# TMElyralab/MuseV

Measured on NVIDIA H100. Metric: denoised frames/sec at 512x512, 16-frame window, 20 DDIM steps, higher is better.
Workload: dtype f16 (fp32 accumulate)

## Files before the change

musev_b200/csrc/conv_gemm.cu:

```cuda
#include "conv_gemm.cuh"

#include <dlfcn.h>
#include <stdio.h>
#include <stdlib.h>
#include <string.h>

#include <mutex>

#include "ptx.cuh"
#include "stats.cuh"

namespace mvb {

static constexpr int kMaxStages = 8;
static constexpr int kBlockM = 128;
static constexpr int kBlockK = 64;
static constexpr int kABytes = kBlockM * kBlockK * 2;
static constexpr int kAccLd = 132;
static constexpr int kAccBytes = 2 * 64 * kAccLd * 4;
static constexpr int kBiasBytes = 2 * 256 * 4;
static constexpr int kRingBytes = 227 * 1024 - kAccBytes - kBiasBytes - 1024  - 256 ;
static constexpr int kSmemBytes = kRingBytes + kAccBytes + kBiasBytes + 1024 + 256;
__device__ __forceinline__ float gelu_erf(float x) { return 0.5f * x * (1.f + erff(x * 0.70710678118654752440f)); }
__device__ __forceinline__ float silu(float x) { return __fdividef(x, 1.f + __expf(-x)); }
__device__ __forceinline__ float gelu_fast(float x) {
  const float z = fabsf(x) * 0.70710678118654752440f;
  const float t = __frcp_rn(fmaf(0.3275911f, z, 1.f));
  float poly = fmaf(1.061405429f, t, -1.453152027f);
  poly = fmaf(poly, t, 1.421413741f);
  poly = fmaf(poly, t, -0.284496736f);
  poly = fmaf(poly, t, 0.254829592f);
  poly *= t;
  float e;
  asm("ex2.approx.ftz.f32 %0, %1;" : "=f"(e) : "f"(-z * z * 1.4426950408889634f));
  const float erf_abs = fmaf(-poly, e, 1.f);
  const float erf_v = copysignf(erf_abs, x);
  return 0.5f * x * (1.f + erf_v);
}

__device__ __forceinline__ float rcp_approx(float x) {
  float y;
  asm("rcp.approx.ftz.f32 %0, %1;" : "=f"(y) : "f"(x));
  return y;
}
__device__ __forceinline__ F2 geglu2(F2 val, F2 gate) {
  float g0, g1;
  f2_get(gate, g0, g1);
  const F2 u = f2_make(fabsf(g0), fabsf(g1));
  float d0, d1;
  f2_get(f2_fma(u, f2_make(0.231641888f, 0.231641888f), f2_make(1.f, 1.f)), d0, d1);
  const F2 t = f2_make(rcp_approx(d0), rcp_approx(d1));
  F2 poly = f2_fma(t, f2_make(-0.5307027145f, -0.5307027145f), f2_make(0.7265760135f, 0.7265760135f));
  poly = f2_fma(poly, t, f2_make(-0.7107068705f, -0.7107068705f));
  poly = f2_fma(poly, t, f2_make(0.142248368f, 0.142248368f));
  poly = f2_fma(poly, t, f2_make(-0.127414796f, -0.127414796f));
  poly = f2_mul(poly, t);
  float a0, a1;
  f2_get(f2_mul(f2_mul(u, f2_make(-0.72134752044f, -0.72134752044f)), u), a0, a1);
  float e0, e1;
  asm("ex2.approx.ftz.f32 %0, %1;" : "=f"(e0) : "f"(a0));
  asm("ex2.approx.ftz.f32 %0, %1;" : "=f"(e1) : "f"(a1));
  const F2 gelu = f2_fma(u, f2_mul(poly, f2_make(e0, e1)), f2_make(fmaxf(g0, 0.f), fmaxf(g1, 0.f)));
  return f2_mul(val, gelu);
}

enum : int {
  kEpiGeneric = 0,
  kEpiPlain = 1,
  kEpiResidual = 2,
  kEpiGeglu = 3,
  kEpiAct = 4
};
__device__ __forceinline__ float gelu_act(float x, int act) {
  return act == 2 ? gelu_erf(x) : act == 3 ? __fdividef(x, 1.f + __expf(-1.702f * x)) : x;
}

struct AMaps {
  CUtensorMap m[4];
};

template <int kEpi, int BN>
__global__ void __launch_bounds__(384, 1)
conv_gemm_kernel(const __grid_constant__ AMaps tmA, const __grid_constant__ CUtensorMap tmB,
                 const __grid_constant__ ConvGemmParams p) {
  extern __shared__ uint8_t smem_raw[];
  uint8_t* smem = reinterpret_cast<uint8_t*>((reinterpret_cast<uintptr_t>(smem_raw) + 1023) & ~uintptr_t(1023));
  float* sacc = reinterpret_cast<float*>(smem + kRingBytes);
  float* sbias = reinterpret_cast<float*>(smem + kRingBytes + kAccBytes);
  uint64_t* bars = reinterpret_cast<uint64_t*>(smem + kRingBytes + kAccBytes + kBiasBytes);
  uint64_t* full = bars;
  uint64_t* empty = bars + kMaxStages;
  const int nstages = p.nstages;
  const int stage_bytes = p.stage_bytes;

  const int warp = threadIdx.x >> 5;
  const int lane = threadIdx.x & 31;

  if (threadIdx.x == 0) {
    tma_prefetch_desc(&tmA.m[0]);
    tma_prefetch_desc(&tmA.m[1]);
    tma_prefetch_desc(&tmA.m[2]);
    tma_prefetch_desc(&tmA.m[3]);
    tma_prefetch_desc(&tmB);
    for (int s = 0; s < kMaxStages; ++s) {
      mbar_init(&full[s], 1);
      mbar_init(&empty[s], 8);
    }
    fence_barrier_init();
  }
  __syncthreads();

  const int kb_per_tap = p.kb0 + p.kb1;
  const int num_kb = p.ntaps * kb_per_tap;
  const int tiles_m = p.tiles_w * p.tiles_h * p.tiles_n;
  const int num_units = tiles_m * p.tiles_nn;
  const uint32_t stage_tx = kABytes + (uint32_t)BN * kBlockK * 2;

  if (warp < 4) {
    setmaxnreg_dec<40>();
    if (warp == 0) {
      int stage = 0;
      uint32_t phase = 0;
      for (int unit = blockIdx.x; unit < num_units; unit += gridDim.x) {
        const int nt = unit % p.tiles_nn;
        const int mt = unit / p.tiles_nn;
        const int tw = mt % p.tiles_w;
        const int th = (mt / p.tiles_w) % p.tiles_h;
        const int tn = mt / (p.tiles_w * p.tiles_h);
        const int w0 = tw * p.bw, h0 = th * p.bh, n0 = tn * p.bn;
        int kcol = 0;
        const int ncoord = nt * BN;
        for (int tap = 0; tap < p.ntaps; ++tap) {
          const int xw = w0 + p.dx[tap], yh = h0 + p.dy[tap];
          const int src0 = p.tap_src[tap];
          for (int cb = 0; cb < kb_per_tap; ++cb, kcol += kBlockK) {
            const bool first = cb < p.kb0;
            const int src = src0 + (first ? 0 : 1);
            const int c0 = (first ? cb : cb - p.kb0) * kBlockK;
            const CUtensorMap* tm = &tmA.m[src];
            mbar_wait(&empty[stage], phase ^ 1);
            if (elect_one()) {
              uint8_t* sa = smem + stage * stage_bytes;
              uint8_t* sb = sa + kABytes;
              mbar_expect_tx(&full[stage], stage_tx);
              tma_load_4d(sa, tm, &full[stage], c0, xw, yh, n0);
              tma_load_2d(sb, &tmB, &full[stage], kcol, ncoord);
            }
            __syncwarp();
            if (++stage == nstages) { stage = 0; phase ^= 1; }
          }
        }
      }
    }
    return;
  }

  setmaxnreg_inc<232>();
  const int wg = (warp - 4) >> 2;
  const int t = threadIdx.x - 128 * (1 + wg);
  const int wq = t >> 5;
  const int row_local = t & 63;
  const int half = t >> 6;
  const int r = 64 * wg + row_local;
  float* acc_slice = sacc + wg * 64 * kAccLd;
  float* wbias = sbias + wg * 256;
  const bool use_res = (p.res != nullptr) && !p.geglu && !p.out_f32;
  const int acc_step = p.geglu ? 64 : 32;
  const uint64_t desc0_a = make_desc_k_sw128(smem_u32(smem) + (uint32_t)wg * 64 * 128);
  const uint64_t desc0_b = make_desc_k_sw128(smem_u32(smem) + kABytes);
  const uint32_t stage_step = (uint32_t)stage_bytes >> 4;
  int stage = 0;
  uint32_t phase = 0;
  float acc[BN / 2];

  for (int unit = blockIdx.x; unit < num_units; unit += gridDim.x) {
    const int nt = unit % p.tiles_nn;
    const int mt = unit / p.tiles_nn;
    const int tw = mt % p.tiles_w;
    const int th = (mt / p.tiles_w) % p.tiles_h;
    const int tn = mt / (p.tiles_w * p.tiles_h);
    const int ncol0 = nt * BN;

    int prev_stage = 0;
    for (int kb = 0; kb < num_kb; ++kb) {
      mbar_wait(&full[stage], phase);
      const uint64_t da = desc0_a + (uint64_t)((uint32_t)stage * stage_step);
      const uint64_t db = desc0_b + (uint64_t)((uint32_t)stage * stage_step);
      wgmma_fence();
      fence_regs(acc);
#pragma unroll
      for (int k = 0; k < kBlockK / 16; ++k)
        Wgmma<BN>::ss(acc, da + (uint64_t)(k * 2), db + (uint64_t)(k * 2), (kb | k) != 0);
      wgmma_commit();
      fence_regs(acc);
      if (kb > 0) {
        wgmma_wait<1>();
        fence_regs(acc);
        __syncwarp();
        if (lane == 0) mbar_arrive(&empty[prev_stage]);
      }
      prev_stage = stage;
      if (++stage == nstages) { stage = 0; phase ^= 1; }
    }
    wgmma_wait<0>();
    fence_regs(acc);
    __syncwarp();
    if (lane == 0) mbar_arrive(&empty[prev_stage]);

    const int rw = r % p.bw;
    const int rh = (r / p.bw) % p.bh;
    const int rn = r / (p.bw * p.bh);
    const int w = tw * p.bw + rw, h = th * p.bh + rh, n = tn * p.bn + rn;
    const bool row_ok = (w < p.W) && (h < p.H) && (n < p.NF);
    const long long m = ((long long)n * p.H + h) * p.W + w;
    const float* radd = (p.rowadd && row_ok) ? p.rowadd + (long long)(m / p.rows_per_group) * p.ld_rowadd : nullptr;
    const __half* res_row = use_res ? p.res + m * p.ld_res : nullptr;
    __half* out_row = reinterpret_cast<__half*>(p.out) + m * p.ldc;

    uint4 rcur[4] = {};
    auto load_res = [&](int c0, uint4 (&dst)[4]) {
      if (!use_res || !row_ok) return;
#pragma unroll
      for (int g = 0; g < 4; ++g) {
        const int nn = ncol0 + c0 + g * 8;
        if (c0 + g * 8 < BN && nn < p.N) dst[g] = __ldg(reinterpret_cast<const uint4*>(res_row + nn));
      }
    };
    named_bar_sync(1 + wg, 128);
    if constexpr (kEpi != kEpiGeneric && kEpi != kEpiAct) {
      for (int c = t; c < BN; c += 128) wbias[c] = (p.bias && ncol0 + c < p.N) ? __ldg(p.bias + ncol0 + c) : 0.f;
    }
#pragma unroll
    for (int u = 0; u < (BN + 127) / 128; ++u) {
      if (u > 0) named_bar_sync(1 + wg, 128);
#pragma unroll
      for (int i = 16 * u; i < 16 * u + 16 && i < BN / 8; ++i) {
        const int rr = 16 * wq + (lane >> 2);
        const int cc = 8 * (i - 16 * u) + 2 * (lane & 3);
        *reinterpret_cast<float2*>(acc_slice + rr * kAccLd + cc) = make_float2(acc[4 * i], acc[4 * i + 1]);
        *reinterpret_cast<float2*>(acc_slice + (rr + 8) * kAccLd + cc) = make_float2(acc[4 * i + 2], acc[4 * i + 3]);
      }
      named_bar_sync(1 + wg, 128);
      const int cend = (128 * u + 128 < BN) ? 128 * u + 128 : BN;
      for (int c0 = 128 * u + half * acc_step; c0 < cend; c0 += 2 * acc_step) {
        const float* srow = acc_slice + row_local * kAccLd + (c0 - 128 * u);
        auto ld32 = [&](const float* src, uint32_t (&v)[32]) {
#pragma unroll
          for (int k = 0; k < 8; ++k) {
            const float4 x = *reinterpret_cast<const float4*>(src + 4 * k);
            v[4 * k] = __float_as_uint(x.x); v[4 * k + 1] = __float_as_uint(x.y);
            v[4 * k + 2] = __float_as_uint(x.z); v[4 * k + 3] = __float_as_uint(x.w);
          }
        };
        load_res(c0, rcur);
        if constexpr (kEpi != kEpiGeneric && kEpi != kEpiAct) {
          const int nbase = ncol0 + c0;
          uint32_t v[32], vg[32];
          ld32(srow, v);
          if constexpr (kEpi == kEpiGeglu) ld32(srow + 32, vg);
          if (nbase < p.N && row_ok) {
            const F2 alpha2 = f2_make(p.alpha, p.alpha);
            const float* cbias = wbias + c0;
            const int oc = (kEpi == kEpiGeglu) ? nbase / 2 : nbase;
#pragma unroll
            for (int g = 0; g < 4; ++g) {
              uint32_t o[4];
              if constexpr (kEpi == kEpiGeglu) {
                const uint32_t* vv = (g < 2) ? v : vg;
                const int j0 = (g & 1) * 8;
#pragma unroll
                for (int e = 0; e < 4; ++e) {
                  const int j = j0 + 2 * e;
                  const float2 bv = *reinterpret_cast<const float2*>(cbias + (g >> 1) * 32 + j);
                  const float2 bg = *reinterpret_cast<const float2*>(cbias + (g >> 1) * 32 + 16 + j);
                  const F2 val = f2_add(f2_make(__uint_as_float(vv[j]), __uint_as_float(vv[j + 1])), f2_make(bv.x, bv.y));
                  const F2 gat = f2_add(f2_make(__uint_as_float(vv[16 + j]), __uint_as_float(vv[16 + j + 1])),
                                        f2_make(bg.x, bg.y));
                  float x0, x1;
                  f2_get(geglu2(val, gat), x0, x1);
                  const __half2 h2 = __floats2half2_rn(x0, x1);
                  o[e] = *reinterpret_cast<const uint32_t*>(&h2);
                }
              } else {
                float4 b0 = *reinterpret_cast<const float4*>(cbias + 8 * g);
                float4 b1 = *reinterpret_cast<const float4*>(cbias + 8 * g + 4);
                if (radd) {
                  const float4 a0 = __ldg(reinterpret_cast<const float4*>(radd + nbase) + 2 * g);
                  const float4 a1 = __ldg(reinterpret_cast<const float4*>(radd + nbase) + 2 * g + 1);
                  b0.x += a0.x; b0.y += a0.y; b0.z += a0.z; b0.w += a0.w;
                  b1.x += a1.x; b1.y += a1.y; b1.z += a1.z; b1.w += a1.w;
                }
                const float bb[8] = {b0.x, b0.y, b0.z, b0.w, b1.x, b1.y, b1.z, b1.w};
                const __half2* rh2 = reinterpret_cast<const __half2*>(&rcur[g]);
#pragma unroll
                for (int e = 0; e < 4; ++e) {
                  const int j = g * 8 + 2 * e;
                  F2 x = f2_add(f2_make(__uint_as_float(v[j]), __uint_as_float(v[j + 1])), f2_make(bb[2 * e], bb[2 * e + 1]));
                  if constexpr (kEpi == kEpiResidual) {
                    const float2 rr = __half22float2(rh2[e]);
                    x = f2_fma(x, alpha2, f2_make(rr.x, rr.y));
                  }
                  float x0, x1;
                  f2_get(x, x0, x1);
                  const __half2 h2 = __floats2half2_rn(x0, x1);
                  o[e] = *reinterpret_cast<const uint32_t*>(&h2);
                }
              }
              *reinterpret_cast<uint4*>(out_row + oc + 8 * g) = make_uint4(o[0], o[1], o[2], o[3]);
            }
          }
        } else {
          float f[32];
          const int nbase = ncol0 + c0;
          if (p.geglu) {
            uint32_t va[32], vb[32];
            ld32(srow, va);
            ld32(srow + 32, vb);
#pragma unroll
            for (int hsel = 0; hsel < 2; ++hsel) {
              const uint32_t* v = hsel ? vb : va;
              const int nb = nbase + hsel * 32;
#pragma unroll
              for (int j4 = 0; j4 < 4; ++j4) {
                const bool bok = p.bias && nb < p.N;
                const float4 bv = bok ? __ldg(reinterpret_cast<const float4*>(p.bias + nb) + j4) : make_float4(0, 0, 0, 0);
                const float4 bg = bok ? __ldg(reinterpret_cast<const float4*>(p.bias + nb + 16) + j4) : make_float4(0, 0, 0, 0);
                const int j = j4 * 4;
                const F2 v01 = f2_add(f2_make(__uint_as_float(v[j]), __uint_as_float(v[j + 1])), f2_make(bv.x, bv.y));
                const F2 v23 = f2_add(f2_make(__uint_as_float(v[j + 2]), __uint_as_float(v[j + 3])), f2_make(bv.z, bv.w));
                const F2 g01 = f2_add(f2_make(__uint_as_float(v[16 + j]), __uint_as_float(v[16 + j + 1])), f2_make(bg.x, bg.y));
                const F2 g23 = f2_add(f2_make(__uint_as_float(v[16 + j + 2]), __uint_as_float(v[16 + j + 3])), f2_make(bg.z, bg.w));
                f2_get(geglu2(v01, g01), f[hsel * 16 + j], f[hsel * 16 + j + 1]);
                f2_get(geglu2(v23, g23), f[hsel * 16 + j + 2], f[hsel * 16 + j + 3]);
              }
            }
          } else {
            uint32_t v[32];
            ld32(srow, v);
            if (nbase + 32 <= p.N) {
#pragma unroll
              for (int g = 0; g < 8; ++g) {
                float4 b = p.bias ? __ldg(reinterpret_cast<const float4*>(p.bias + nbase) + g) : make_float4(0, 0, 0, 0);
                if (radd) {
                  const float4 a4 = __ldg(reinterpret_cast<const float4*>(radd + nbase) + g);
                  b.x += a4.x; b.y += a4.y; b.z += a4.z; b.w += a4.w;
                }
                f[g * 4 + 0] = __uint_as_float(v[g * 4 + 0]) + b.x;
                f[g * 4 + 1] = __uint_as_float(v[g * 4 + 1]) + b.y;
                f[g * 4 + 2] = __uint_as_float(v[g * 4 + 2]) + b.z;
                f[g * 4 + 3] = __uint_as_float(v[g * 4 + 3]) + b.w;
              }
            } else {
#pragma unroll
              for (int j = 0; j < 32; ++j) {
                const int nn = nbase + j;
                float x = __uint_as_float(v[j]);
                if (nn < p.N) {
                  if (p.bias) x += __ldg(p.bias + nn);
                  if (radd) x += __ldg(radd + nn);
                }
                f[j] = x;
              }
            }
          }
          if (row_ok) {
            if (p.out_f32) {
#pragma unroll
              for (int g = 0; g < 8; ++g) {
                const int nn = nbase + g * 4;
                if (nn < p.N) {
                  float4 o4;
                  o4.x = f[g * 4 + 0] * p.alpha; o4.y = f[g * 4 + 1] * p.alpha;
                  o4.z = f[g * 4 + 2] * p.alpha; o4.w = f[g * 4 + 3] * p.alpha;
                  if (p.act == 1) { o4.x = silu(o4.x); o4.y = silu(o4.y); o4.z = silu(o4.z); o4.w = silu(o4.w); }
                  if constexpr (kEpi == kEpiAct) {
                    o4.x = gelu_act(o4.x, p.act); o4.y = gelu_act(o4.y, p.act);
                    o4.z = gelu_act(o4.z, p.act); o4.w = gelu_act(o4.w, p.act);
                  }
                  *reinterpret_cast<float4*>(reinterpret_cast<float*>(p.out) + m * p.ldc + nn) = o4;
                }
              }
            } else {
              const int oc = p.geglu ? nbase / 2 : nbase;
              const int ncols = p.geglu ? p.N / 2 : p.N;
#pragma unroll
              for (int g = 0; g < 4; ++g) {
                if (oc + 8 * g >= ncols) continue;
                __align__(16) __half o[8];
                const __half* rh8 = reinterpret_cast<const __half*>(&rcur[g]);
#pragma unroll
                for (int j = 0; j < 8; ++j) {
                  float x = f[g * 8 + j];
                  if (!p.geglu) {
                    x *= p.alpha;
                    if (use_res) x = fmaf(p.beta, __half2float(rh8[j]), x);
                    if (p.act == 1) x = silu(x);
                    if constexpr (kEpi == kEpiAct) x = gelu_act(x, p.act);
                  }
                  o[j] = __float2half_rn(x);
                }
                *reinterpret_cast<uint4*>(out_row + oc + 8 * g) = *reinterpret_cast<const uint4*>(o);
              }
            }
          }
        }
      }
    }
  }
}

typedef CUresult (*EncodeTiledFn)(CUtensorMap*, CUtensorMapDataType, cuuint32_t, void*, const cuuint64_t*,
                                  const cuuint64_t*, const cuuint32_t*, const cuuint32_t*, CUtensorMapInterleave,
                                  CUtensorMapSwizzle, CUtensorMapL2promotion, CUtensorMapFloatOOBfill);

EncodeTiledFn get_encode_fn() {
  static EncodeTiledFn fn = nullptr;
  static bool tried = false;
  if (!tried) {
    tried = true;
    void* h = dlopen("libcuda.so.1", RTLD_NOW | RTLD_GLOBAL);
    if (!h) h = dlopen("libcuda.so", RTLD_NOW | RTLD_GLOBAL);
    if (h) fn = reinterpret_cast<EncodeTiledFn>(dlsym(h, "cuTensorMapEncodeTiled"));
  }
  return fn;
}

namespace {
struct MapKey {
  uint64_t ptr, d[4], s[3];
  uint32_t box[4], rank, swz;
  bool operator==(const MapKey& o) const { return memcmp(this, &o, sizeof(MapKey)) == 0; }
};
struct MapSlot {
  MapKey key;
  CUtensorMap map;
  bool used;
};
static_assert(sizeof(MapKey) == 88, "MapKey is compared and hashed bytewise: no padding allowed");
static_assert(sizeof(MapSlot) % 64 == 0, "slots keep the 64-byte alignment of CUtensorMap");
constexpr uint32_t kMapSlots = 1u << 14;
std::mutex g_map_mutex;
MapSlot* g_map_slots = nullptr;
uint32_t g_map_count = 0;
unsigned long long g_map_hits = 0, g_map_misses = 0;

uint64_t hash_key(const MapKey& k) {
  const uint64_t* w = reinterpret_cast<const uint64_t*>(&k);
  uint64_t h = 0x9e3779b97f4a7c15ull;
  for (size_t i = 0; i < sizeof(MapKey) / 8; ++i) {
    h ^= w[i] + 0x9e3779b97f4a7c15ull + (h << 6) + (h >> 2);
    h *= 0xff51afd7ed558ccdull;
    h ^= h >> 33;
  }
  return h;
}
bool cache_enabled() {
  static const bool on = !(getenv("MVB_TMAP_CACHE") && atoi(getenv("MVB_TMAP_CACHE")) == 0);
  return on;
}
// ... 92 lines not shown
      }
    }
  }
}

static const int kBlockNs[4] = {64, 128, 160, 256};

static int pick_block_n(int N, int geglu, int gelu, long long tiles_m, int num_sms) {
  int best = 0;
  double best_cost = 1e30;
  for (int i = 3; i >= 0; --i) {
    const int bn = kBlockNs[i];
    if (geglu && (bn % 64)) continue;
    if (gelu && bn == 256) continue;
    const int tn = ceil_div(N, bn);
    const long long tiles = tiles_m * tn;
    const long long waves = (tiles + num_sms - 1) / num_sms;
    const double cost = (double)waves * (bn + 24.0);
    if (cost < best_cost - 1e-9) { best_cost = cost; best = bn; }
  }
  return best;
}

static cudaError_t launch_common(cudaStream_t stream, const CUtensorMap* maps, int nmaps, ConvGemmParams& p,
                                 const __half* wt, long long ktot, const Epilogue& ep, int num_sms, const char** err) {
  typedef void (*KernelFn)(const AMaps, const CUtensorMap, const ConvGemmParams);
#define MVB_GEMM_ROW(BN) \
  {conv_gemm_kernel<kEpiGeneric, BN>, conv_gemm_kernel<kEpiPlain, BN>, conv_gemm_kernel<kEpiResidual, BN>, \
   conv_gemm_kernel<kEpiGeglu, BN>, conv_gemm_kernel<kEpiAct, BN>}
  static const KernelFn kernels[4][5] = {MVB_GEMM_ROW(64), MVB_GEMM_ROW(128), MVB_GEMM_ROW(160),
                                         {conv_gemm_kernel<kEpiGeneric, 256>, conv_gemm_kernel<kEpiPlain, 256>,
                                          conv_gemm_kernel<kEpiResidual, 256>, conv_gemm_kernel<kEpiGeglu, 256>, nullptr}};
#undef MVB_GEMM_ROW
  static bool attr_set_dev[64] = {};
  int cur_dev = 0;
  cudaGetDevice(&cur_dev);
  bool& attr_set = attr_set_dev[cur_dev & 63];
  if (!attr_set) {
    for (int a = 0; a < 4; ++a)
      for (int b = 0; b < 5; ++b) {
        if (!kernels[a][b]) continue;
        cudaError_t e = cudaFuncSetAttribute(reinterpret_cast<const void*>(kernels[a][b]),
                                             cudaFuncAttributeMaxDynamicSharedMemorySize, kSmemBytes);
        if (e != cudaSuccess) { *err = "cudaFuncSetAttribute(conv_gemm_kernel)"; return e; }
      }
    attr_set = true;
  }
  const long long tiles_m = (long long)p.tiles_w * p.tiles_h * p.tiles_n;
  const int gelu = ep.act == 2 || ep.act == 3;
  p.block_n = pick_block_n(p.N, ep.geglu, gelu, tiles_m, num_sms);
  int bn_idx = 0;
  while (kBlockNs[bn_idx] != p.block_n) ++bn_idx;
  p.tiles_nn = ceil_div(p.N, p.block_n);
  p.stage_bytes = kABytes + ((p.block_n * kBlockK * 2 + 1023) / 1024) * 1024;
  p.nstages = kRingBytes / p.stage_bytes;
  if (p.nstages > kMaxStages) p.nstages = kMaxStages;
  p.out = ep.out; p.ldc = ep.ldc; p.bias = ep.bias; p.rowadd = ep.rowadd;
  p.rows_per_group = ep.rows_per_group > 0 ? ep.rows_per_group : 1;
  p.ld_rowadd = ep.ld_rowadd; p.res = ep.res; p.ld_res = ep.ld_res; p.alpha = ep.alpha; p.beta = ep.beta;
  p.geglu = ep.geglu; p.act = ep.act; p.out_f32 = ep.out_f32;
  if (ep.out_f32 && (ep.geglu || ep.res)) { *err = "conv_gemm: fp32 output excludes geglu/residual"; return cudaErrorInvalidValue; }
  if ((ep.ldc % (ep.out_f32 ? 4 : 8)) || (reinterpret_cast<uintptr_t>(ep.out) % 16)) {
    *err = "conv_gemm: the output must be 16-byte aligned with a row stride of whole 16-byte vectors";
    return cudaErrorInvalidValue;
  }
  CUtensorMap tmB;
  if (!encode_map_2d(&tmB, wt, (uint64_t)ktot, (uint64_t)p.N, (uint64_t)ktot, 64u, (uint32_t)p.block_n)) {
    *err = "cuTensorMapEncodeTiled(B) failed";
    return cudaErrorInvalidValue;
  }
  const long long num_tiles = tiles_m * p.tiles_nn;
  const int grid = (int)(num_tiles < num_sms ? num_tiles : num_sms);
  int epi = kEpiGeneric;
  if (!ep.out_f32 && ep.act == 0) {
    if (ep.geglu) { if (p.N % 64 == 0 && !ep.rowadd) epi = kEpiGeglu; }
    else if (p.N % 32 == 0) {
      if (ep.res && ep.beta == 1.f) epi = kEpiResidual;
      else if (!ep.res && ep.alpha == 1.f) epi = kEpiPlain;
    }
  }
  if (gelu) epi = kEpiAct;
  static const bool trace = getenv("MVB_TRACE") != nullptr;
  if (trace)
    fprintf(stderr, "MVB_TRACE gemm M=%lld N=%d K=%lld taps=%d block_n=%d tiles=%lld geglu=%d res=%d f32=%d epi=%d\n",
            (long long)p.W * p.H * p.NF, p.N, ktot, p.ntaps, p.block_n, num_tiles, p.geglu, p.res != nullptr, p.out_f32,
            epi);
  AMaps am;
  for (int i = 0; i < 4; ++i) am.m[i] = maps[i < nmaps ? i : 0];
  ProfScope prof(stream, KC_GEMM);
  kernels[bn_idx][epi]<<<grid, 384, kSmemBytes, stream>>>(am, tmB, p);
  cudaError_t e = cudaGetLastError();
  if (e != cudaSuccess) *err = "conv_gemm_kernel launch";
  return e;
}

cudaError_t launch_conv_gemm(cudaStream_t stream, const ASource& a0, const ASource* a1, int W, int H, int NF,
                             int ntaps, const int8_t* dy, const int8_t* dx, const __half* wt, int N,
                             const Epilogue& ep, int num_sms, const char** err) {
  if ((a0.C % 64) || (a1 && (a1->C % 64)) || (N % 8) || ntaps < 1 || ntaps > 9) {
    *err = "conv_gemm: channels must be multiples of 64, N a multiple of 8, 1..9 taps";
    return cudaErrorInvalidValue;
  }
  ConvGemmParams p{};
  p.W = W; p.H = H; p.NF = NF;
  pick_box(W, H, NF, &p.bw, &p.bh, &p.bn);
  p.tiles_w = ceil_div(W, p.bw); p.tiles_h = ceil_div(H, p.bh); p.tiles_n = ceil_div(NF, p.bn);
  p.ntaps = ntaps;
  for (int i = 0; i < ntaps; ++i) { p.dy[i] = dy[i]; p.dx[i] = dx[i]; p.tap_src[i] = 0; }
  p.kb0 = a0.C / 64;
  p.kb1 = a1 ? a1->C / 64 : 0;
  p.N = N;
  CUtensorMap maps[2];
  const uint32_t box[4] = {64u, (uint32_t)p.bw, (uint32_t)p.bh, (uint32_t)p.bn};
  {
    const uint64_t dims[4] = {(uint64_t)a0.C, (uint64_t)W, (uint64_t)H, (uint64_t)NF};
    const uint64_t st[3] = {(uint64_t)a0.sW, (uint64_t)a0.sH, (uint64_t)a0.sN};
    if (!encode_map_4d(&maps[0], a0.ptr, dims, st, box)) { *err = "cuTensorMapEncodeTiled(A0) failed"; return cudaErrorInvalidValue; }
  }
  if (a1) {
    const uint64_t dims[4] = {(uint64_t)a1->C, (uint64_t)W, (uint64_t)H, (uint64_t)NF};
    const uint64_t st[3] = {(uint64_t)a1->sW, (uint64_t)a1->sH, (uint64_t)a1->sN};
    if (!encode_map_4d(&maps[1], a1->ptr, dims, st, box)) { *err = "cuTensorMapEncodeTiled(A1) failed"; return cudaErrorInvalidValue; }
  }
  const long long ktot = (long long)ntaps * (a0.C + (a1 ? a1->C : 0));
  return launch_common(stream, maps, a1 ? 2 : 1, p, wt, ktot, ep, num_sms, err);
}

cudaError_t launch_conv_s2(cudaStream_t stream, const __half* x, int C, int W, int H, int NF, const __half* wt, int N,
                           const Epilogue& ep, int num_sms, const char** err, int pad_mode) {
  if ((C % 64) || (N % 8) || (W % 2) || (H % 2)) {
    *err = "conv_s2: channels multiple of 64, even H and W";
    return cudaErrorInvalidValue;
  }
  if (pad_mode != 1 && pad_mode != 2) {
    *err = "conv_s2: pad mode must be 1 (pad 1 on every side) or 2 (pad (0, 1, 0, 1))";
    return cudaErrorInvalidValue;
  }
  const int Wo = W / 2, Ho = H / 2;
  ConvGemmParams p{};
  p.W = Wo; p.H = Ho; p.NF = NF;
  pick_box(Wo, Ho, NF, &p.bw, &p.bh, &p.bn);
  p.tiles_w = ceil_div(Wo, p.bw); p.tiles_h = ceil_div(Ho, p.bh); p.tiles_n = ceil_div(NF, p.bn);
  p.ntaps = 9;
// ... 26 lines not shown
```

Measured before the change: 5.112.

## Add dedicated epilogue warpgroup to overlap conv GEMM epilogue with next tile's MMA

For tile widths up to 160, the conv GEMM kernel now launches 512 threads, with a fourth warpgroup that owns the epilogue. The consumer warpgroups write their accumulators into a swizzled fp32 staging buffer and signal through acc_full/acc_empty mbarriers, then go straight on to the next tile's MMAs while the epilogue warpgroup applies bias, residual and activation and stores the result. This hides epilogue time behind the main loop. In exchange, consumer registers drop to 152, the staging buffer takes shared memory from the pipeline ring (stage counts are now fixed per width), and BN=256 keeps the old inline path.

Result: faster. 5.348, median of 6 (+4.6%).

```diff
diff --git a/musev_b200/csrc/conv_gemm.cu b/musev_b200/csrc/conv_gemm.cu
--- a/musev_b200/csrc/conv_gemm.cu
+++ b/musev_b200/csrc/conv_gemm.cu
@@ -16,11 +16,22 @@
 static constexpr int kBlockM = 128;
 static constexpr int kBlockK = 64;
 static constexpr int kABytes = kBlockM * kBlockK * 2;
+static constexpr int kSmemBytes = 227 * 1024;
+constexpr bool inline_epilogue(int bn) { return bn == 256; }
+constexpr int conv_threads(int bn) { return inline_epilogue(bn) ? 384 : 512; }
+static constexpr int kMaxStagedN = 160;
+static constexpr int kStagingBytes = kBlockM * kMaxStagedN * 4;
 static constexpr int kAccLd = 132;
 static constexpr int kAccBytes = 2 * 64 * kAccLd * 4;
-static constexpr int kBiasBytes = 2 * 256 * 4;
-static constexpr int kRingBytes = 227 * 1024 - kAccBytes - kBiasBytes - 1024  - 256 ;
-static constexpr int kSmemBytes = kRingBytes + kAccBytes + kBiasBytes + 1024 + 256;
+constexpr int epi_buf_bytes(int bn) { return inline_epilogue(bn) ? kAccBytes : kStagingBytes; }
+constexpr int bias_buf_bytes(int bn) { return inline_epilogue(bn) ? 2 * 256 * 4 : kMaxStagedN * 4; }
+constexpr int ring_bytes(int bn) { return kSmemBytes - epi_buf_bytes(bn) - bias_buf_bytes(bn) - 1024  - 256 ; }
+constexpr int ring_stage_bytes(int bn) { return kABytes + (bn * kBlockK * 2 + 1023) / 1024 * 1024; }
+constexpr int ring_stages(int bn) {
+  return ring_bytes(bn) / ring_stage_bytes(bn) < kMaxStages ? ring_bytes(bn) / ring_stage_bytes(bn) : kMaxStages;
+}
+static_assert(ring_stages(64) == 6 && ring_stages(128) == 4 && ring_stages(160) == 4 && ring_stages(256) == 3,
+              "shared-memory budget per tile width");
 __device__ __forceinline__ float gelu_erf(float x) { return 0.5f * x * (1.f + erff(x * 0.70710678118654752440f)); }
 __device__ __forceinline__ float silu(float x) { return __fdividef(x, 1.f + __expf(-x)); }
 __device__ __forceinline__ float gelu_fast(float x) {
@@ -79,17 +90,251 @@
   CUtensorMap m[4];
 };
 
+template <int kEpi, class Ld>
+__device__ __forceinline__ void finish_run(const ConvGemmParams& p, const Ld& ld32, int c0, int ncol0, const float* sbias,
+                                           const float* radd, const uint4 (&rcur)[4], bool row_ok, bool use_res,
+                                           long long m, __half* out_row) {
+  if constexpr (kEpi != kEpiGeneric && kEpi != kEpiAct) {
+    const int nbase = ncol0 + c0;
+    uint32_t v[32], vg[32];
+    ld32(c0, v);
+    if constexpr (kEpi == kEpiGeglu) ld32(c0 + 32, vg);
+    if (nbase < p.N && row_ok) {
+      const F2 alpha2 = f2_make(p.alpha, p.alpha);
+      const float* cbias = sbias + c0;
+      const int oc = (kEpi == kEpiGeglu) ? nbase / 2 : nbase;
+#pragma unroll
+      for (int g = 0; g < 4; ++g) {
+        uint32_t o[4];
+        if constexpr (kEpi == kEpiGeglu) {
+          const uint32_t* vv = (g < 2) ? v : vg;
+          const int j0 = (g & 1) * 8;
+#pragma unroll
+          for (int e = 0; e < 4; ++e) {
+            const int j = j0 + 2 * e;
+            const float2 bv = *reinterpret_cast<const float2*>(cbias + (g >> 1) * 32 + j);
+            const float2 bg = *reinterpret_cast<const float2*>(cbias + (g >> 1) * 32 + 16 + j);
+            const F2 val = f2_add(f2_make(__uint_as_float(vv[j]), __uint_as_float(vv[j + 1])), f2_make(bv.x, bv.y));
+            const F2 gat = f2_add(f2_make(__uint_as_float(vv[16 + j]), __uint_as_float(vv[16 + j + 1])),
+                                  f2_make(bg.x, bg.y));
+            float x0, x1;
+            f2_get(geglu2(val, gat), x0, x1);
+            const __half2 h2 = __floats2half2_rn(x0, x1);
+            o[e] = *reinterpret_cast<const uint32_t*>(&h2);
+          }
+        } else {
+          float4 b0 = *reinterpret_cast<const float4*>(cbias + 8 * g);
+          float4 b1 = *reinterpret_cast<const float4*>(cbias + 8 * g + 4);
+          if (radd) {
+            const float4 a0 = __ldg(reinterpret_cast<const float4*>(radd + nbase) + 2 * g);
+            const float4 a1 = __ldg(reinterpret_cast<const float4*>(radd + nbase) + 2 * g + 1);
+            b0.x += a0.x; b0.y += a0.y; b0.z += a0.z; b0.w += a0.w;
+            b1.x += a1.x; b1.y += a1.y; b1.z += a1.z; b1.w += a1.w;
+          }
+          const float bb[8] = {b0.x, b0.y, b0.z, b0.w, b1.x, b1.y, b1.z, b1.w};
+          const __half2* rh2 = reinterpret_cast<const __half2*>(&rcur[g]);
+#pragma unroll
+          for (int e = 0; e < 4; ++e) {
+            const int j = g * 8 + 2 * e;
+            F2 x = f2_add(f2_make(__uint_as_float(v[j]), __uint_as_float(v[j + 1])), f2_make(bb[2 * e], bb[2 * e + 1]));
+            if constexpr (kEpi == kEpiResidual) {
+              const float2 rr = __half22float2(rh2[e]);
+              x = f2_fma(x, alpha2, f2_make(rr.x, rr.y));
+            }
+            float x0, x1;
+            f2_get(x, x0, x1);
+            const __half2 h2 = __floats2half2_rn(x0, x1);
+            o[e] = *reinterpret_cast<const uint32_t*>(&h2);
+          }
+        }
+        *reinterpret_cast<uint4*>(out_row + oc + 8 * g) = make_uint4(o[0], o[1], o[2], o[3]);
+      }
+    }
+  } else {
+    float f[32];
+    const int nbase = ncol0 + c0;
+    if (p.geglu) {
+      uint32_t va[32], vb[32];
+      ld32(c0, va);
+      ld32(c0 + 32, vb);
+#pragma unroll
+      for (int hsel = 0; hsel < 2; ++hsel) {
+        const uint32_t* v = hsel ? vb : va;
+        const int nb = nbase + hsel * 32;
+#pragma unroll
+        for (int j4 = 0; j4 < 4; ++j4) {
+          const bool bok = p.bias && nb < p.N;
+          const float4 bv = bok ? __ldg(reinterpret_cast<const float4*>(p.bias + nb) + j4) : make_float4(0, 0, 0, 0);
+          const float4 bg = bok ? __ldg(reinterpret_cast<const float4*>(p.bias + nb + 16) + j4) : make_float4(0, 0, 0, 0);
+          const int j = j4 * 4;
+          const F2 v01 = f2_add(f2_make(__uint_as_float(v[j]), __uint_as_float(v[j + 1])), f2_make(bv.x, bv.y));
+          const F2 v23 = f2_add(f2_make(__uint_as_float(v[j + 2]), __uint_as_float(v[j + 3])), f2_make(bv.z, bv.w));
+          const F2 g01 = f2_add(f2_make(__uint_as_float(v[16 + j]), __uint_as_float(v[16 + j + 1])), f2_make(bg.x, bg.y));
+          const F2 g23 = f2_add(f2_make(__uint_as_float(v[16 + j + 2]), __uint_as_float(v[16 + j + 3])), f2_make(bg.z, bg.w));
+          f2_get(geglu2(v01, g01), f[hsel * 16 + j], f[hsel * 16 + j + 1]);
+          f2_get(geglu2(v23, g23), f[hsel * 16 + j + 2], f[hsel * 16 + j + 3]);
+        }
+      }
+    } else {
+      uint32_t v[32];
+      ld32(c0, v);
+      if (nbase + 32 <= p.N) {
+#pragma unroll
+        for (int g = 0; g < 8; ++g) {
+          float4 b = p.bias ? __ldg(reinterpret_cast<const float4*>(p.bias + nbase) + g) : make_float4(0, 0, 0, 0);
+          if (radd) {
+            const float4 a4 = __ldg(reinterpret_cast<const float4*>(radd + nbase) + g);
+            b.x += a4.x; b.y += a4.y; b.z += a4.z; b.w += a4.w;
+          }
+          f[g * 4 + 0] = __uint_as_float(v[g * 4 + 0]) + b.x;
+          f[g * 4 + 1] = __uint_as_float(v[g * 4 + 1]) + b.y;
+          f[g * 4 + 2] = __uint_as_float(v[g * 4 + 2]) + b.z;
+          f[g * 4 + 3] = __uint_as_float(v[g * 4 + 3]) + b.w;
+        }
+      } else {
+#pragma unroll
+        for (int j = 0; j < 32; ++j) {
+          const int nn = nbase + j;
+          float x = __uint_as_float(v[j]);
+          if (nn < p.N) {
+            if (p.bias) x += __ldg(p.bias + nn);
+            if (radd) x += __ldg(radd + nn);
+          }
+          f[j] = x;
+        }
+      }
+    }
+    if (row_ok) {
+      if (p.out_f32) {
+#pragma unroll
+        for (int g = 0; g < 8; ++g) {
+          const int nn = nbase + g * 4;
+          if (nn < p.N) {
+            float4 o4;
+            o4.x = f[g * 4 + 0] * p.alpha; o4.y = f[g * 4 + 1] * p.alpha;
+            o4.z = f[g * 4 + 2] * p.alpha; o4.w = f[g * 4 + 3] * p.alpha;
+            if (p.act == 1) { o4.x = silu(o4.x); o4.y = silu(o4.y); o4.z = silu(o4.z); o4.w = silu(o4.w); }
+            if constexpr (kEpi == kEpiAct) {
+              o4.x = gelu_act(o4.x, p.act); o4.y = gelu_act(o4.y, p.act);
+              o4.z = gelu_act(o4.z, p.act); o4.w = gelu_act(o4.w, p.act);
+            }
+            *reinterpret_cast<float4*>(reinterpret_cast<float*>(p.out) + m * p.ldc + nn) = o4;
+          }
+        }
+      } else {
+        const int oc = p.geglu ? nbase / 2 : nbase;
+        const int ncols = p.geglu ? p.N / 2 : p.N;
+#pragma unroll
+        for (int g = 0; g < 4; ++g) {
+          if (oc + 8 * g >= ncols) continue;
+          __align__(16) __half o[8];
+          const __half* rh8 = reinterpret_cast<const __half*>(&rcur[g]);
+#pragma unroll
+          for (int j = 0; j < 8; ++j) {
+            float x = f[g * 8 + j];
+            if (!p.geglu) {
+              x *= p.alpha;
+              if (use_res) x = fmaf(p.beta, __half2float(rh8[j]), x);
+              if (p.act == 1) x = silu(x);
+              if constexpr (kEpi == kEpiAct) x = gelu_act(x, p.act);
+            }
+            o[j] = __float2half_rn(x);
+          }
+          *reinterpret_cast<uint4*>(out_row + oc + 8 * g) = *reinterpret_cast<const uint4*>(o);
+        }
+      }
+    }
+  }
+}
+
 template <int kEpi, int BN>
-__global__ void __launch_bounds__(384, 1)
+__device__ __forceinline__ void inline_epilogue_tile(const ConvGemmParams& p, const float (&acc)[BN / 2], float* sacc,
+                                                     float* sbias, int unit, int wg, int t) {
+  const int lane = t & 31;
+  const int wq = t >> 5;
+  const int row_local = t & 63;
+  const int half = t >> 6;
+  const int r = 64 * wg + row_local;
+  float* acc_slice = sacc + wg * 64 * kAccLd;
+  float* wbias = sbias + wg * 256;
+  const bool use_res = (p.res != nullptr) && !p.geglu && !p.out_f32;
+  const int acc_step = p.geglu ? 64 : 32;
+  const int nt = unit % p.tiles_nn;
+  const int mt = unit / p.tiles_nn;
+  const int tw = mt % p.tiles_w;
+  const int th = (mt / p.tiles_w) % p.tiles_h;
+  const int tn = mt / (p.tiles_w * p.tiles_h);
+  const int ncol0 = nt * BN;
+  const int rw = r % p.bw;
+  const int rh = (r / p.bw) % p.bh;
+  const int rn = r / (p.bw * p.bh);
+  const int w = tw * p.bw + rw, h = th * p.bh + rh, n = tn * p.bn + rn;
+  const bool row_ok = (w < p.W) && (h < p.H) && (n < p.NF);
+  const long long m = ((long long)n * p.H + h) * p.W + w;
+  const float* radd = (p.rowadd && row_ok) ? p.rowadd + (long long)(m / p.rows_per_group) * p.ld_rowadd : nullptr;
+  const __half* res_row = use_res ? p.res + m * p.ld_res : nullptr;
+  __half* out_row = reinterpret_cast<__half*>(p.out) + m * p.ldc;
+
+  uint4 rcur[4] = {};
+  auto load_res = [&](int c0) {
+    if (!use_res || !row_ok) return;
+#pragma unroll
+    for (int g = 0; g < 4; ++g) {
+      const int nn = ncol0 + c0 + g * 8;
+      if (c0 + g * 8 < BN && nn < p.N) rcur[g] = __ldg(reinterpret_cast<const uint4*>(res_row + nn));
+    }
+  };
+  named_bar_sync(1 + wg, 128);
+  if constexpr (kEpi != kEpiGeneric && kEpi != kEpiAct) {
+    for (int c = t; c < BN; c += 128) wbias[c] = (p.bias && ncol0 + c < p.N) ? __ldg(p.bias + ncol0 + c) : 0.f;
+  }
+#pragma unroll
+  for (int u = 0; u < (BN + 127) / 128; ++u) {
+    if (u > 0) named_bar_sync(1 + wg, 128);
+#pragma unroll
+    for (int i = 16 * u; i < 16 * u + 16 && i < BN / 8; ++i) {
+      const int rr = 16 * wq + (lane >> 2);
+      const int cc = 8 * (i - 16 * u) + 2 * (lane & 3);
+      *reinterpret_cast<float2*>(acc_slice + rr * kAccLd + cc) = make_float2(acc[4 * i], acc[4 * i + 1]);
+      *reinterpret_cast<float2*>(acc_slice + (rr + 8) * kAccLd + cc) = make_float2(acc[4 * i + 2], acc[4 * i + 3]);
+    }
+    named_bar_sync(1 + wg, 128);
+    const int cend = (128 * u + 128 < BN) ? 128 * u + 128 : BN;
+    for (int c0 = 128 * u + half * acc_step; c0 < cend; c0 += 2 * acc_step) {
+      const float* srow = acc_slice + row_local * kAccLd - 128 * u;
+      auto ld32 = [&](int col, uint32_t (&v)[32]) {
+#pragma unroll
+        for (int k = 0; k < 8; ++k) {
+          const float4 x = *reinterpret_cast<const float4*>(srow + col + 4 * k);
+          v[4 * k] = __float_as_uint(x.x); v[4 * k + 1] = __float_as_uint(x.y);
+          v[4 * k + 2] = __float_as_uint(x.z); v[4 * k + 3] = __float_as_uint(x.w);
+        }
+      };
+      load_res(c0);
+      finish_run<kEpi>(p, ld32, c0, ncol0, wbias, radd, rcur, row_ok, use_res, m, out_row);
+    }
+  }
+}
+
+template <int kEpi, int BN>
+__global__ void __launch_bounds__(conv_threads(BN), 1)
 conv_gemm_kernel(const __grid_constant__ AMaps tmA, const __grid_constant__ CUtensorMap tmB,
                  const __grid_constant__ ConvGemmParams p) {
+  constexpr bool kInline = inline_epilogue(BN);
+  static_assert(BN % 32 == 0 && (BN <= kMaxStagedN || kInline), "the staging swizzle and the epilogue take whole 32-column runs");
+  constexpr int kProducerRegs = 40, kConsumerRegs = kInline ? 232 : 152, kEpilogueRegs = kInline ? 0 : 168;
+  static_assert(128 * (kProducerRegs + kEpilogueRegs) + 256 * kConsumerRegs <= 65536,
+                "setmaxnreg split exceeds the register file");
+  constexpr int kRingBytes = ring_bytes(BN);
   extern __shared__ uint8_t smem_raw[];
   uint8_t* smem = reinterpret_cast<uint8_t*>((reinterpret_cast<uintptr_t>(smem_raw) + 1023) & ~uintptr_t(1023));
-  float* sacc = reinterpret_cast<float*>(smem + kRingBytes);
-  float* sbias = reinterpret_cast<float*>(smem + kRingBytes + kAccBytes);
-  uint64_t* bars = reinterpret_cast<uint64_t*>(smem + kRingBytes + kAccBytes + kBiasBytes);
+  float* stg = reinterpret_cast<float*>(smem + kRingBytes);
+  float* sbias = reinterpret_cast<float*>(smem + kRingBytes + epi_buf_bytes(BN));
+  uint64_t* bars = reinterpret_cast<uint64_t*>(smem + kRingBytes + epi_buf_bytes(BN) + bias_buf_bytes(BN));
   uint64_t* full = bars;
   uint64_t* empty = bars + kMaxStages;
+  uint64_t* acc_full = bars + 2 * kMaxStages;
+  uint64_t* acc_empty = acc_full + 1;
   const int nstages = p.nstages;
   const int stage_bytes = p.stage_bytes;
 
@@ -106,6 +351,8 @@
       mbar_init(&full[s], 1);
       mbar_init(&empty[s], 8);
     }
+    mbar_init(acc_full, 8);
+    mbar_init(acc_empty, 4);
     fence_barrier_init();
   }
   __syncthreads();
@@ -117,7 +364,7 @@
   const uint32_t stage_tx = kABytes + (uint32_t)BN * kBlockK * 2;
 
   if (warp < 4) {
-    setmaxnreg_dec<40>();
+    setmaxnreg_dec<kProducerRegs>();
     if (warp == 0) {
       int stage = 0;
       uint32_t phase = 0;
@@ -155,32 +402,85 @@
     return;
   }
 
-  setmaxnreg_inc<232>();
+  if (!kInline && warp >= 12) {
+    setmaxnreg_inc<kEpilogueRegs>();
+    const int r = threadIdx.x - 384;
+    const float* srow = stg + r * BN;
+    const int sw = r & 7;
+    const bool use_res = (p.res != nullptr) && !p.geglu && !p.out_f32;
+    const int acc_step = p.geglu ? 64 : 32;
+    uint32_t acc_phase = 0;
+    for (int unit = blockIdx.x; unit < num_units; unit += gridDim.x) {
+      const int nt = unit % p.tiles_nn;
+      const int mt = unit / p.tiles_nn;
+      const int tw = mt % p.tiles_w;
+      const int th = (mt / p.tiles_w) % p.tiles_h;
+      const int tn = mt / (p.tiles_w * p.tiles_h);
+      const int ncol0 = nt * BN;
+      const int rw = r % p.bw;
+      const int rh = (r / p.bw) % p.bh;
+      const int rn = r / (p.bw * p.bh);
+      const int w = tw * p.bw + rw, h = th * p.bh + rh, n = tn * p.bn + rn;
+      const bool row_ok = (w < p.W) && (h < p.H) && (n < p.NF);
+      const long long m = ((long long)n * p.H + h) * p.W + w;
+      const float* radd = (p.rowadd && row_ok) ? p.rowadd + (long long)(m / p.rows_per_group) * p.ld_rowadd : nullptr;
+      const __half* res_row = use_res ? p.res + m * p.ld_res : nullptr;
+      __half* out_row = reinterpret_cast<__half*>(p.out) + m * p.ldc;
+
+      uint4 rcur[4] = {}, rnext[4] = {};
+      auto load_res = [&](int c0, uint4 (&dst)[4]) {
+        if (!use_res || !row_ok) return;
+#pragma unroll
+        for (int g = 0; g < 4; ++g) {
+          const int nn = ncol0 + c0 + g * 8;
+          if (c0 + g * 8 < BN && nn < p.N) dst[g] = __ldg(reinterpret_cast<const uint4*>(res_row + nn));
+        }
+      };
+      if constexpr (kEpi != kEpiGeneric && kEpi != kEpiAct) {
+        named_bar_sync(1, 128);
+        for (int c = r; c < BN; c += 128) sbias[c] = (p.bias && ncol0 + c < p.N) ? __ldg(p.bias + ncol0 + c) : 0.f;
+        named_bar_sync(1, 128);
+      }
+      load_res(0, rcur);
+      mbar_wait(acc_full, acc_phase);
+      for (int c0 = 0; c0 < BN; c0 += acc_step) {
+        if constexpr (kEpi == kEpiResidual) load_res(c0 + acc_step, rnext);
+        else if (c0 > 0) load_res(c0, rcur);
+        auto ld32 = [&](int col, uint32_t (&v)[32]) {
+#pragma unroll
+          for (int k = 0; k < 8; ++k) {
+            const float4 x = *reinterpret_cast<const float4*>(srow + col + 4 * (k ^ sw));
+            v[4 * k] = __float_as_uint(x.x); v[4 * k + 1] = __float_as_uint(x.y);
+            v[4 * k + 2] = __float_as_uint(x.z); v[4 * k + 3] = __float_as_uint(x.w);
+          }
+        };
+        finish_run<kEpi>(p, ld32, c0, ncol0, sbias, radd, rcur, row_ok, use_res, m, out_row);
+        if constexpr (kEpi == kEpiResidual) {
+#pragma unroll
+          for (int g = 0; g < 4; ++g) rcur[g] = rnext[g];
+        }
+      }
+      __syncwarp();
+      if (lane == 0) mbar_arrive(acc_empty);
+      acc_phase ^= 1;
+    }
+    return;
+  }
+
+  setmaxnreg_inc<kConsumerRegs>();
   const int wg = (warp - 4) >> 2;
   const int t = threadIdx.x - 128 * (1 + wg);
   const int wq = t >> 5;
-  const int row_local = t & 63;
-  const int half = t >> 6;
-  const int r = 64 * wg + row_local;
-  float* acc_slice = sacc + wg * 64 * kAccLd;
-  float* wbias = sbias + wg * 256;
-  const bool use_res = (p.res != nullptr) && !p.geglu && !p.out_f32;
-  const int acc_step = p.geglu ? 64 : 32;
   const uint64_t desc0_a = make_desc_k_sw128(smem_u32(smem) + (uint32_t)wg * 64 * 128);
   const uint64_t desc0_b = make_desc_k_sw128(smem_u32(smem) + kABytes);
   const uint32_t stage_step = (uint32_t)stage_bytes >> 4;
+  float* stg_row = stg + (64 * wg + 16 * wq + (lane >> 2)) * BN;
   int stage = 0;
   uint32_t phase = 0;
+  uint32_t acc_phase = 0;
   float acc[BN / 2];
 
   for (int unit = blockIdx.x; unit < num_units; unit += gridDim.x) {
-    const int nt = unit % p.tiles_nn;
-    const int mt = unit / p.tiles_nn;
-    const int tw = mt % p.tiles_w;
-    const int th = (mt / p.tiles_w) % p.tiles_h;
-    const int tn = mt / (p.tiles_w * p.tiles_h);
-    const int ncol0 = nt * BN;
-
     int prev_stage = 0;
     for (int kb = 0; kb < num_kb; ++kb) {
       mbar_wait(&full[stage], phase);
@@ -207,204 +507,19 @@
     __syncwarp();
     if (lane == 0) mbar_arrive(&empty[prev_stage]);
 
-    const int rw = r % p.bw;
-    const int rh = (r / p.bw) % p.bh;
-    const int rn = r / (p.bw * p.bh);
-    const int w = tw * p.bw + rw, h = th * p.bh + rh, n = tn * p.bn + rn;
-    const bool row_ok = (w < p.W) && (h < p.H) && (n < p.NF);
-    const long long m = ((long long)n * p.H + h) * p.W + w;
-    const float* radd = (p.rowadd && row_ok) ? p.rowadd + (long long)(m / p.rows_per_group) * p.ld_rowadd : nullptr;
-    const __half* res_row = use_res ? p.res + m * p.ld_res : nullptr;
-    __half* out_row = reinterpret_cast<__half*>(p.out) + m * p.ldc;
-
-    uint4 rcur[4] = {};
-    auto load_res = [&](int c0, uint4 (&dst)[4]) {
-      if (!use_res || !row_ok) return;
-#pragma unroll
-      for (int g = 0; g < 4; ++g) {
-        const int nn = ncol0 + c0 + g * 8;
-        if (c0 + g * 8 < BN && nn < p.N) dst[g] = __ldg(reinterpret_cast<const uint4*>(res_row + nn));
-      }
-    };
-    named_bar_sync(1 + wg, 128);
-    if constexpr (kEpi != kEpiGeneric && kEpi != kEpiAct) {
-      for (int c = t; c < BN; c += 128) wbias[c] = (p.bias && ncol0 + c < p.N) ? __ldg(p.bias + ncol0 + c) : 0.f;
-    }
-#pragma unroll
-    for (int u = 0; u < (BN + 127) / 128; ++u) {
-      if (u > 0) named_bar_sync(1 + wg, 128);
-#pragma unroll
-      for (int i = 16 * u; i < 16 * u + 16 && i < BN / 8; ++i) {
-        const int rr = 16 * wq + (lane >> 2);
-        const int cc = 8 * (i - 16 * u) + 2 * (lane & 3);
-        *reinterpret_cast<float2*>(acc_slice + rr * kAccLd + cc) = make_float2(acc[4 * i], acc[4 * i + 1]);
-        *reinterpret_cast<float2*>(acc_slice + (rr + 8) * kAccLd + cc) = make_float2(acc[4 * i + 2], acc[4 * i + 3]);
-      }
-      named_bar_sync(1 + wg, 128);
-      const int cend = (128 * u + 128 < BN) ? 128 * u + 128 : BN;
-      for (int c0 = 128 * u + half * acc_step; c0 < cend; c0 += 2 * acc_step) {
-        const float* srow = acc_slice + row_local * kAccLd + (c0 - 128 * u);
-        auto ld32 = [&](const float* src, uint32_t (&v)[32]) {
-#pragma unroll
-          for (int k = 0; k < 8; ++k) {
-            const float4 x = *reinterpret_cast<const float4*>(src + 4 * k);
-            v[4 * k] = __float_as_uint(x.x); v[4 * k + 1] = __float_as_uint(x.y);
-            v[4 * k + 2] = __float_as_uint(x.z); v[4 * k + 3] = __float_as_uint(x.w);
-          }
-        };
-        load_res(c0, rcur);
-        if constexpr (kEpi != kEpiGeneric && kEpi != kEpiAct) {
-          const int nbase = ncol0 + c0;
-          uint32_t v[32], vg[32];
-          ld32(srow, v);
-          if constexpr (kEpi == kEpiGeglu) ld32(srow + 32, vg);
-          if (nbase < p.N && row_ok) {
-            const F2 alpha2 = f2_make(p.alpha, p.alpha);
-            const float* cbias = wbias + c0;
-            const int oc = (kEpi == kEpiGeglu) ? nbase / 2 : nbase;
-#pragma unroll
-            for (int g = 0; g < 4; ++g) {
-              uint32_t o[4];
-              if constexpr (kEpi == kEpiGeglu) {
-                const uint32_t* vv = (g < 2) ? v : vg;
-                const int j0 = (g & 1) * 8;
-#pragma unroll
-                for (int e = 0; e < 4; ++e) {
-                  const int j = j0 + 2 * e;
-                  const float2 bv = *reinterpret_cast<const float2*>(cbias + (g >> 1) * 32 + j);
-                  const float2 bg = *reinterpret_cast<const float2*>(cbias + (g >> 1) * 32 + 16 + j);
-                  const F2 val = f2_add(f2_make(__uint_as_float(vv[j]), __uint_as_float(vv[j + 1])), f2_make(bv.x, bv.y));
-                  const F2 gat = f2_add(f2_make(__uint_as_float(vv[16 + j]), __uint_as_float(vv[16 + j + 1])),
-                                        f2_make(bg.x, bg.y));
-                  float x0, x1;
-                  f2_get(geglu2(val, gat), x0, x1);
-                  const __half2 h2 = __floats2half2_rn(x0, x1);
-                  o[e] = *reinterpret_cast<const uint32_t*>(&h2);
-                }
-              } else {
-                float4 b0 = *reinterpret_cast<const float4*>(cbias + 8 * g);
-                float4 b1 = *reinterpret_cast<const float4*>(cbias + 8 * g + 4);
-                if (radd) {
-                  const float4 a0 = __ldg(reinterpret_cast<const float4*>(radd + nbase) + 2 * g);
-                  const float4 a1 = __ldg(reinterpret_cast<const float4*>(radd + nbase) + 2 * g + 1);
-                  b0.x += a0.x; b0.y += a0.y; b0.z += a0.z; b0.w += a0.w;
-                  b1.x += a1.x; b1.y += a1.y; b1.z += a1.z; b1.w += a1.w;
-                }
-                const float bb[8] = {b0.x, b0.y, b0.z, b0.w, b1.x, b1.y, b1.z, b1.w};
-                const __half2* rh2 = reinterpret_cast<const __half2*>(&rcur[g]);
-#pragma unroll
-                for (int e = 0; e < 4; ++e) {
-                  const int j = g * 8 + 2 * e;
-                  F2 x = f2_add(f2_make(__uint_as_float(v[j]), __uint_as_float(v[j + 1])), f2_make(bb[2 * e], bb[2 * e + 1]));
-                  if constexpr (kEpi == kEpiResidual) {
-                    const float2 rr = __half22float2(rh2[e]);
-                    x = f2_fma(x, alpha2, f2_make(rr.x, rr.y));
-                  }
-                  float x0, x1;
-                  f2_get(x, x0, x1);
-                  const __half2 h2 = __floats2half2_rn(x0, x1);
-                  o[e] = *reinterpret_cast<const uint32_t*>(&h2);
-                }
-              }
-              *reinterpret_cast<uint4*>(out_row + oc + 8 * g) = make_uint4(o[0], o[1], o[2], o[3]);
-            }
-          }
-        } else {
-          float f[32];
-          const int nbase = ncol0 + c0;
-          if (p.geglu) {
-            uint32_t va[32], vb[32];
-            ld32(srow, va);
-            ld32(srow + 32, vb);
-#pragma unroll
-            for (int hsel = 0; hsel < 2; ++hsel) {
-              const uint32_t* v = hsel ? vb : va;
-              const int nb = nbase + hsel * 32;
-#pragma unroll
-              for (int j4 = 0; j4 < 4; ++j4) {
-                const bool bok = p.bias && nb < p.N;
-                const float4 bv = bok ? __ldg(reinterpret_cast<const float4*>(p.bias + nb) + j4) : make_float4(0, 0, 0, 0);
-                const float4 bg = bok ? __ldg(reinterpret_cast<const float4*>(p.bias + nb + 16) + j4) : make_float4(0, 0, 0, 0);
-                const int j = j4 * 4;
-                const F2 v01 = f2_add(f2_make(__uint_as_float(v[j]), __uint_as_float(v[j + 1])), f2_make(bv.x, bv.y));
-                const F2 v23 = f2_add(f2_make(__uint_as_float(v[j + 2]), __uint_as_float(v[j + 3])), f2_make(bv.z, bv.w));
-                const F2 g01 = f2_add(f2_make(__uint_as_float(v[16 + j]), __uint_as_float(v[16 + j + 1])), f2_make(bg.x, bg.y));
-                const F2 g23 = f2_add(f2_make(__uint_as_float(v[16 + j + 2]), __uint_as_float(v[16 + j + 3])), f2_make(bg.z, bg.w));
-                f2_get(geglu2(v01, g01), f[hsel * 16 + j], f[hsel * 16 + j + 1]);
-                f2_get(geglu2(v23, g23), f[hsel * 16 + j + 2], f[hsel * 16 + j + 3]);
-              }
-            }
-          } else {
-            uint32_t v[32];
-            ld32(srow, v);
-            if (nbase + 32 <= p.N) {
-#pragma unroll
-              for (int g = 0; g < 8; ++g) {
-                float4 b = p.bias ? __ldg(reinterpret_cast<const float4*>(p.bias + nbase) + g) : make_float4(0, 0, 0, 0);
-                if (radd) {
-                  const float4 a4 = __ldg(reinterpret_cast<const float4*>(radd + nbase) + g);
-                  b.x += a4.x; b.y += a4.y; b.z += a4.z; b.w += a4.w;
-                }
-                f[g * 4 + 0] = __uint_as_float(v[g * 4 + 0]) + b.x;
-                f[g * 4 + 1] = __uint_as_float(v[g * 4 + 1]) + b.y;
-                f[g * 4 + 2] = __uint_as_float(v[g * 4 + 2]) + b.z;
-                f[g * 4 + 3] = __uint_as_float(v[g * 4 + 3]) + b.w;
-              }
-            } else {
-#pragma unroll
-              for (int j = 0; j < 32; ++j) {
-                const int nn = nbase + j;
-                float x = __uint_as_float(v[j]);
-                if (nn < p.N) {
-                  if (p.bias) x += __ldg(p.bias + nn);
-                  if (radd) x += __ldg(radd + nn);
-                }
-                f[j] = x;
-              }
-            }
-          }
-          if (row_ok) {
-            if (p.out_f32) {
-#pragma unroll
-              for (int g = 0; g < 8; ++g) {
-                const int nn = nbase + g * 4;
-                if (nn < p.N) {
-                  float4 o4;
-                  o4.x = f[g * 4 + 0] * p.alpha; o4.y = f[g * 4 + 1] * p.alpha;
-                  o4.z = f[g * 4 + 2] * p.alpha; o4.w = f[g * 4 + 3] * p.alpha;
-                  if (p.act == 1) { o4.x = silu(o4.x); o4.y = silu(o4.y); o4.z = silu(o4.z); o4.w = silu(o4.w); }
-                  if constexpr (kEpi == kEpiAct) {
-                    o4.x = gelu_act(o4.x, p.act); o4.y = gelu_act(o4.y, p.act);
-                    o4.z = gelu_act(o4.z, p.act); o4.w = gelu_act(o4.w, p.act);
-                  }
-                  *reinterpret_cast<float4*>(reinterpret_cast<float*>(p.out) + m * p.ldc + nn) = o4;
-                }
-              }
-            } else {
-              const int oc = p.geglu ? nbase / 2 : nbase;
-              const int ncols = p.geglu ? p.N / 2 : p.N;
-#pragma unroll
-              for (int g = 0; g < 4; ++g) {
-                if (oc + 8 * g >= ncols) continue;
-                __align__(16) __half o[8];
-                const __half* rh8 = reinterpret_cast<const __half*>(&rcur[g]);
-#pragma unroll
-                for (int j = 0; j < 8; ++j) {
-                  float x = f[g * 8 + j];
-                  if (!p.geglu) {
-                    x *= p.alpha;
-                    if (use_res) x = fmaf(p.beta, __half2float(rh8[j]), x);
-                    if (p.act == 1) x = silu(x);
-                    if constexpr (kEpi == kEpiAct) x = gelu_act(x, p.act);
-                  }
-                  o[j] = __float2half_rn(x);
-                }
-                *reinterpret_cast<uint4*>(out_row + oc + 8 * g) = *reinterpret_cast<const uint4*>(o);
-              }
-            }
-          }
-        }
-      }
+    if constexpr (kInline) {
+      inline_epilogue_tile<kEpi, BN>(p, acc, stg, sbias, unit, wg, t);
+    } else {
+      mbar_wait(acc_empty, acc_phase ^ 1);
+#pragma unroll
+      for (int i = 0; i < BN / 8; ++i) {
+        const int off = 4 * ((2 * i + ((lane & 3) >> 1)) ^ (lane >> 2)) + 2 * (lane & 1);
+        *reinterpret_cast<float2*>(stg_row + off) = make_float2(acc[4 * i], acc[4 * i + 1]);
+        *reinterpret_cast<float2*>(stg_row + 8 * BN + off) = make_float2(acc[4 * i + 2], acc[4 * i + 3]);
+      }
+      __syncwarp();
+      if (lane == 0) mbar_arrive(acc_full);
+      acc_phase ^= 1;
     }
   }
 }
@@ -603,9 +718,8 @@
   int bn_idx = 0;
   while (kBlockNs[bn_idx] != p.block_n) ++bn_idx;
   p.tiles_nn = ceil_div(p.N, p.block_n);
-  p.stage_bytes = kABytes + ((p.block_n * kBlockK * 2 + 1023) / 1024) * 1024;
-  p.nstages = kRingBytes / p.stage_bytes;
-  if (p.nstages > kMaxStages) p.nstages = kMaxStages;
+  p.stage_bytes = ring_stage_bytes(p.block_n);
+  p.nstages = ring_stages(p.block_n);
   p.out = ep.out; p.ldc = ep.ldc; p.bias = ep.bias; p.rowadd = ep.rowadd;
   p.rows_per_group = ep.rows_per_group > 0 ? ep.rows_per_group : 1;
   p.ld_rowadd = ep.ld_rowadd; p.res = ep.res; p.ld_res = ep.ld_res; p.alpha = ep.alpha; p.beta = ep.beta;
@@ -632,14 +746,22 @@
   }
   if (gelu) epi = kEpiAct;
   static const bool trace = getenv("MVB_TRACE") != nullptr;
-  if (trace)
-    fprintf(stderr, "MVB_TRACE gemm M=%lld N=%d K=%lld taps=%d block_n=%d tiles=%lld geglu=%d res=%d f32=%d epi=%d\n",
+  if (trace) {
+    char taps[9 * 10 + 1];
+    int len = 0;
+    for (int i = 0; i < p.ntaps; ++i) len += snprintf(taps + len, sizeof(taps) - len, "%s%d:%d", i ? "," : "", p.dy[i], p.dx[i]);
+    int s2 = 0;
+    for (int i = 0; i < p.ntaps; ++i) if (p.tap_src[i]) s2 = p.dy[0] < 0 ? 1 : 2;
+    fprintf(stderr, "MVB_TRACE gemm M=%lld N=%d K=%lld taps=%d block_n=%d tiles=%lld geglu=%d res=%d f32=%d epi=%d "
+            "W=%d H=%d NF=%d c0=%d c1=%d offsets=%s s2=%d bias=%d rowadd=%d rpg=%d alpha=%.9g beta=%.9g act=%d\n",
             (long long)p.W * p.H * p.NF, p.N, ktot, p.ntaps, p.block_n, num_tiles, p.geglu, p.res != nullptr, p.out_f32,
-            epi);
+            epi, p.W, p.H, p.NF, p.kb0 * 64, p.kb1 * 64, taps, s2, p.bias != nullptr, p.rowadd != nullptr,
+            p.rows_per_group, p.alpha, p.beta, p.act);
+  }
   AMaps am;
   for (int i = 0; i < 4; ++i) am.m[i] = maps[i < nmaps ? i : 0];
   ProfScope prof(stream, KC_GEMM);
-  kernels[bn_idx][epi]<<<grid, 384, kSmemBytes, stream>>>(am, tmB, p);
+  kernels[bn_idx][epi]<<<grid, conv_threads(p.block_n), kSmemBytes, stream>>>(am, tmB, p);
   cudaError_t e = cudaGetLastError();
   if (e != cudaSuccess) *err = "conv_gemm_kernel launch";
   return e;
```
